# OpenDriveLab/MTGS

Hardware: AMD Instinct MI355X
Metric: rendered Mpix/s (fwd+bwd) @ 2M Gaussians 1920x1080 (higher is better)
Workload: dtype f32

## Files before the change

### include/mtgs_rast.h

```cpp
#ifndef MTGS_RAST_H
#define MTGS_RAST_H

#include <stddef.h>
#include <stdint.h>

#include "mtgs_crop.h"
#include "mtgs_refine_scene.h"
#include "mtgs_present.h"
#include "mtgs_lpips.h"
#include "mtgs_dino.h"
#include "mtgs_jpeg.h"
#include "mtgs_lidar.h"
#include "mtgs_frame.h"
#include "mtgs_stack.h"
#include "mtgs_jpegdec.h"
#include "mtgs_icp.h"

#ifdef __cplusplus
extern "C" {
#endif

#define MTGS_RAST_ABI_VERSION 29
#define MTGS_RAST_HOT_ABI_VERSION 7
#define MTGS_VIS_COLOR_ROWS 64
#define MTGS_BIN3_TIGHT 1
#define MTGS_BIN3_FILL_TO_M 2
#define MTGS_BIN3_FILL_TO_CAP 4
#define MTGS_BIN3_PREZEROED 8
#define MTGS_BIN3_STATUS 16

enum {
    MTGS_OK = 0,
    MTGS_EINVAL = 1,
    MTGS_ELAUNCH = 2,
    MTGS_EWORKSPACE = 3,
    MTGS_EUNSUPPORTED = 4
};

#define MTGS_TILE_SIZE 16
// ... 465 lines not shown
```

### mtgs_amd/_lib.py

```python
from __future__ import annotations

import ctypes as C
from pathlib import Path

import torch

from . import _abi

_PKG = Path(__file__).resolve().parent
LIB_PATH = _PKG / "libmtgs_rast.so"


def use_library(path) -> None:
    global LIB_PATH
    if _lib is not None:
        raise RuntimeError("use_library() after the library was loaded")
    LIB_PATH = Path(path)

_PROTOTYPES = {_abi.HEADER.name: _abi.prototypes()}
for _name in _abi.included_headers():
    _PROTOTYPES[_name] = _abi.header_abi(_name).prototypes
GROUPS = {header: list(group) for header, group in _PROTOTYPES.items()}
EXPORTS = GROUPS[_abi.HEADER.name]
ABI_VERSION = _abi.constant("MTGS_RAST_ABI_VERSION")
# ... 18 lines not shown
            fn.restype = restype
    v = lib.mtgs_rast_version()
    if v != ABI_VERSION:
        raise RuntimeError(f"libmtgs_rast.so ABI version {v} != expected {ABI_VERSION}; rebuild")
    if lib.mtgs_rast_hot_version() != HOT_ABI_VERSION:
        raise RuntimeError(f"libmtgs_rast.so hot-path ABI version {lib.mtgs_rast_hot_version()} != expected {HOT_ABI_VERSION}; rebuild")
    _lib = lib
    return lib


def ptr(t):
    return None if t is None else t.data_ptr()


def host_i64(values):
    return None if values is None else (C.c_int64 * len(values))(*values)


def stream_of(t: torch.Tensor):
    return torch.cuda.current_stream(t.device).cuda_stream


_timed: dict = {}


def time_calls(names=()) -> None:
    _timed.clear()
    for n in names:
        _timed[n] = []


def timed_ms() -> dict:
    return {n: [s.elapsed_time(e) for s, e in evs] for n, evs in _timed.items()}


def call(name: str, *args) -> None:
    evs = _timed.get(name) if _timed else None
    if evs is not None:
        s, e = torch.cuda.Event(enable_timing=True), torch.cuda.Event(enable_timing=True)
        s.record()
    rc = getattr(load(), name)(*args)
    if evs is not None:
        e.record()
        evs.append((s, e))
    if rc != 0:
        msg = load().mtgs_rast_last_error().decode("utf-8", "replace")
        raise RuntimeError(f"{name} failed (code {rc}): {msg}")


def size_query(name: str, *dims) -> int:
    n = C.c_size_t(0)
    call(name, *dims, C.byref(n))
    return n.value


def workspace(name: str, *dims, device, dtype, pad: int = 0) -> torch.Tensor:
    return torch.empty(size_query(name, *dims) + pad, dtype=dtype, device=device)


_scratch: dict = {}
# ... 17 lines not shown
```

### mtgs_amd/csrc/blend.hip

```cpp
#include <stdlib.h>
#include <type_traits>
#include "common.hpp"
#include "wave_reduce.hpp"
#include "raster_rec.hpp"

#ifdef MTGS_DEV
#include "dev/blend_dev.hpp"
#else
#define MTGS_COUNT_ADD(i, v) do { } while (0)
#define MTGS_COUNT_SLOTS(vmask) do { } while (0)
#define MTGS_DEV_PPL_OVERRIDE() do { } while (0)
#define MTGS_TL_DECL() do { } while (0)
#define MTGS_TL_STAGED(n) do { } while (0)
#define MTGS_TL_ACTIVE() do { } while (0)
#define MTGS_TL_END(kind) do { } while (0)
#endif

namespace {

constexpr float kAlphaMax = MTGS_ALPHA_MAX;
constexpr float kTMin = MTGS_T_MIN;
constexpr float kNoClampOpacity = 0.9989f;
constexpr float kHalfLog2e = MTGS_HALF_LOG2E;

// ... 189 lines not shown
extern "C" int mtgs_fill_zero(void *p, size_t bytes, void *stream);
inline int zero_fill_fallback(void *&also_zero, size_t also_zero_bytes, int64_t tiles, hipStream_t st) {
    if (!also_zero || also_zero_bytes == 0 || also_zero_bytes / (size_t)(tiles > 0 ? tiles : 1) <= ZERO_FILL_MAX_PER_TILE) return MTGS_OK;
    void *p = also_zero;
    also_zero = nullptr;
    return mtgs_fill_zero(p, also_zero_bytes, (void *)st);
}
inline ZeroFill make_zero_fill(void *also_zero, size_t also_zero_bytes, unsigned grid, int waves_per_block) {
    ZeroFill zf{nullptr, 0ull, 0u};
    if (also_zero && also_zero_bytes) {
        const unsigned long long n16 = also_zero_bytes / 16, waves = (unsigned long long)grid * waves_per_block;
        zf = ZeroFill{(uint4 *)also_zero, n16, (uint32_t)((n16 + waves - 1) / waves)};
    }
    return zf;
}

template <int D, int PPL, bool PK>
__global__ __launch_bounds__(256 / PPL, (PPL == 4 && D <= 4) ? MTGS_FWD_WAVES : 1) void blend_fwd_kernel(
    int C, const float *__restrict__ recs, const float *__restrict__ means2d, const float *__restrict__ conics,
    const float *__restrict__ colors, const float *__restrict__ opacities,
    const float *__restrict__ backgrounds, const float *__restrict__ depths, int DC, int ed, int W, int H,
    int tw, int th, const int32_t *__restrict__ offsets, const int32_t *__restrict__ flatten_ids, int64_t M,
    float *__restrict__ render, float *__restrict__ alphas, int32_t *__restrict__ last_ids,
    const int32_t *__restrict__ order, const ZeroFill zf) {
    constexpr int NT = 256 / PPL, ROWS = NT / 16, REC = Rec<D>::N;
    constexpr bool CULL = true;
    constexpr int CAND = NT == 64 ? 128 : 256, NR = CAND / NT;
    __shared__ __attribute__((aligned(16))) float s_rec[CAND * REC];
    __shared__ int s_wc[NT / 64];
    MTGS_TL_DECL();
    const int64_t n_tiles = (int64_t)tw * th, total_tiles = (int64_t)C * n_tiles;
    const int64_t tile = block_to_tile(order);
    const int cam = (int)(tile / n_tiles);
    const int t_in = (int)(tile - (int64_t)cam * n_tiles);
    const int ty = t_in / tw, tx = t_in - ty * tw;
    const int tid = threadIdx.x, lx = tid & 15, ly = tid >> 4;
    const int ix = tx * 16 + lx;
    const float px = (float)ix + 0.5f;
    int iy[PPL];
    float py[PPL], T[PPL], acc[PPL][D];
    int32_t last[PPL];
    unsigned long long done[PPL];
    bool inside[PPL];
#pragma unroll
    for (int p = 0; p < PPL; ++p) {
        iy[p] = ty * 16 + ly + p * ROWS;
        py[p] = (float)iy[p] + 0.5f;
        inside[p] = ix < W && iy[p] < H;
        done[p] = __ballot(!inside[p]);
        T[p] = 1.f;
        last[p] = 0;
#pragma unroll
        for (int k = 0; k < D; ++k) acc[p][k] = 0.f;
// ... 23 lines not shown
        for (int r = 0; r < NR; ++r)
            if (b0 + CAND + r * NT + tid < end) g_next[r] = flatten_ids[b0 + CAND + r * NT + tid];
        __syncthreads();
        auto entry = [&](const float4 &r0, const float4 &r1, const uint32_t va, auto off_tag, auto clamp_tag) -> bool {
            constexpr int OFF = decltype(off_tag)::value;
            constexpr bool CLAMP = decltype(clamp_tag)::value;
            ColorRow<D, REC> col;
            col.template load_at<OFF * REC * 4>(va, py[0]);
            const float dx = r0.x - px;
            const float adx = r0.z * dx, bdx = r0.w * dx;
            const float q0 = adx * dx, b2dx = bdx + bdx;
            float s2[PPL];
            unsigned long long vmask[PPL], any = 0;
#pragma unroll
            for (int p = 0; p < PPL; ++p) {
                s2[p] = eval_s2(q0, b2dx, r1.x, r0.y - py[p]);
                vmask[p] = in_range_mask(s2[p], r1.z) & ~done[p];
                any |= vmask[p];
            }
            col.wait();
            if (any == 0) return false;
            MTGS_TL_ACTIVE();
            const int32_t idx = __float_as_int(r1.w);
            unsigned long long stopped = 0;
#pragma unroll
            for (int p = 0; p < PPL; ++p) {
                if (vmask[p] != 0) {
                    const float e = __builtin_amdgcn_exp2f(-s2[p]);
                    const float alpha = CLAMP ? fminf(kAlphaMax, alpha_rounded(r1.y, e)) : alpha_rounded(r1.y, e);
                    const float w = alpha * T[p];
                    const float next_T = T[p] * (1.f - alpha);
                    const unsigned long long sm = __builtin_amdgcn_fcmpf(next_T, kTMin, 5 ) & vmask[p];
                    done[p] |= sm;
                    stopped |= sm;
                    const bool upd = __builtin_amdgcn_inverse_ballot_w64(vmask[p] & ~sm);
                    const float wu = upd ? w : 0.f;
#pragma unroll
                    for (int k = 0; k < D; ++k) acc[p][k] = fmaf(col[k], wu, acc[p][k]);
                    T[p] = upd ? next_T : T[p];
                    last[p] = upd ? idx : last[p];
                }
            }
            if (stopped) {
                unsigned long long ad = done[0];
#pragma unroll
                for (int p = 1; p < PPL; ++p) ad &= done[p];
                return ad == ~0ull;
            }
            return false;
        };
        auto run = [&](auto clamp_tag) {
            using Z = std::integral_constant<int, 0>;
            using O = std::integral_constant<int, 1>;
            const uint32_t rec0 = lds_offset(s_rec);
            auto rec_at = [&](uint32_t va, int q) {
                const f32x4 v = *reinterpret_cast<const __attribute__((address_space(3))) f32x4 *>((uintptr_t)(va + 16 * q));
                return make_float4(v.x, v.y, v.z, v.w);
            };
            uint32_t va;
            asm volatile("v_mov_b32 %0, %1" : "=v"(va) : "s"(rec0));
            float4 ra0 = rec_at(va, 0), ra1 = rec_at(va, 1), rb0 = ra0, rb1 = ra1;
            bool fin = false;
            for (int t = 0; t < bsz && !fin; t += 2) {
                asm volatile("v_mov_b32 %0, %1" : "=v"(va) : "s"(rec0 + (uint32_t)t * (REC * 4)));
                if (t + 1 < bsz) { rb0 = rec_at(va, REC / 4); rb1 = rec_at(va, REC / 4 + 1); }
                fin = entry(ra0, ra1, va, Z{}, clamp_tag);
// ... 1 lines not shown
                    if (t + 2 < bsz) { ra0 = rec_at(va, 2 * (REC / 4)); ra1 = rec_at(va, 2 * (REC / 4) + 1); }
                    fin = entry(rb0, rb1, va, O{}, clamp_tag);
                }
            }
        };
        if (may_clamp) run(std::true_type{}); else run(std::false_type{});
    }
#pragma unroll
    for (int p = 0; p < PPL; ++p) {
        if (inside[p]) {
            const int64_t pid = ((int64_t)cam * H + iy[p]) * W + ix;
            const float alpha_out = 1.f - T[p];
            alphas[pid] = alpha_out;
            last_ids[pid] = last[p];
#pragma unroll
            for (int k = 0; k < D; ++k) {
                float v = (backgrounds && k < DC) ? acc[p][k] + T[p] * backgrounds[cam * DC + k] : acc[p][k];
                if (ed && k == D - 1) v = v / fmaxf(alpha_out, 1e-10f);
                render[pid * D + k] = v;
            }
        }
    }
    zero_fill_slice<NT>(zf);
    MTGS_TL_END(0);
}

template <int PPL>
__global__ __launch_bounds__(256 / PPL) void blend_touch_kernel(int C, const float *__restrict__ recs, int W, int H, int tw, int th,
                                                                const int32_t *__restrict__ offsets,
                                                                const int32_t *__restrict__ rank_ids,
                                                                const int32_t *__restrict__ order, uint8_t *__restrict__ touched) {
    constexpr int NT = 256 / PPL, ROWS = NT / 16, REC = Rec<0>::N;
    constexpr int CAND = NT == 64 ? 128 : 256, NR = CAND / NT;
    static_assert(REC == 8, "geometry half of the record");
    __shared__ __attribute__((aligned(16))) float s_rec[CAND * REC];
    __shared__ int32_t s_id[CAND];
    __shared__ int s_wc[NT / 64];
    const int64_t n_tiles = (int64_t)tw * th;
    const int64_t tile = block_to_tile(order);
    const int cam = (int)(tile / n_tiles);
    const int t_in = (int)(tile - (int64_t)cam * n_tiles);
    const int ty = t_in / tw, tx = t_in - ty * tw;
    const int tid = threadIdx.x, lx = tid & 15, ly = tid >> 4;
    const int ix = tx * 16 + lx;
    const float px = (float)ix + 0.5f;
    float py[PPL], T[PPL];
// ... 319 lines not shown
            }
        };
        if (may_clamp) run(std::true_type{}); else run(std::false_type{});
        if (BATCH_FLUSH) {
            __syncthreads();
            for (int e = tid; e < bsz * 16; e += NT) {
                const int t = e >> 4;
                float v = 0.f;
#pragma unroll
                for (int w = 0; w < NW; ++w) v += s_grad[(w * CAND + t) * 16 + j];
                if (a_base && v != 0.f) unsafeAtomicAdd(row_address(a_base, (uint32_t)s_id[t], a_stride_bytes), v);
            }
        }
    }
    zero_slice();
}

template <int D, int PPL, bool PK = false>
int launch_fwd(int C, const float *recs, const float *means2d, const float *conics, const float *colors,
               const float *opacities, const float *backgrounds, const float *depths, int DC, int ed, int W,
               int H, int tw, int th,
               const int32_t *offsets, const int32_t *flatten_ids, int64_t M, float *render,
               float *alphas, int32_t *last_ids, const int32_t *order, hipStream_t st, void *also_zero = nullptr,
               size_t also_zero_bytes = 0) {
    const int64_t total = (int64_t)C * tw * th;
    const unsigned grid = (unsigned)total;
    blend_fwd_kernel<D, PPL, PK><<<grid, 256 / PPL, 0, st>>>(C, recs, means2d, conics, colors, opacities,
                                                         backgrounds, depths, DC, ed, W, H, tw, th, offsets,
                                                         flatten_ids, M, render, alphas, last_ids, order,
                                                         make_zero_fill(also_zero, also_zero_bytes, grid, 256 / PPL / 64));
    return 0;
}

template <int D, int PPL, bool PK = false>
int launch_bwd(int C, const float *recs, const float *means2d, const float *conics, const float *colors,
               const float *opacities, const float *backgrounds, const float *depths, int DC, int ed, int W,
               int H, int tw, int th, const int32_t *offsets, const int32_t *flatten_ids, int64_t M,
               const float *alphas, const int32_t *last_ids, const float *render, const float *v_render,
               const float *v_alphas, float *v_means2d, float *v_means2d_abs, float *v_conics, float *v_colors,
               float *v_depths, float *v_opacities, const GradRowBytes gs, const int32_t *row_index, const int32_t *order,
               hipStream_t st, void *also_zero = nullptr, size_t also_zero_bytes = 0) {
    const int64_t total = (int64_t)C * tw * th;
    const unsigned grid = (unsigned)total;
    const ZeroFill zf = make_zero_fill(also_zero, also_zero_bytes, grid, 256 / PPL / 64);
    blend_bwd_kernel<D, PPL, PK><<<grid, 256 / PPL, 0, st>>>(
        C, recs, means2d, conics, colors, opacities, backgrounds, depths, DC, ed, W, H, tw, th, offsets, flatten_ids, M,
        alphas, last_ids, render, v_render, v_alphas, v_means2d, v_means2d_abs, v_conics, v_colors, v_depths,
        v_opacities, gs, row_index, order, zf);
    return 0;
}

constexpr int SCHED_THREADS = 1024, SCHED_BUCKETS = 1024;
__global__ __launch_bounds__(SCHED_THREADS) void tile_schedule_kernel(int total_tiles, const int32_t *__restrict__ offsets,
                                                                     int64_t M, int32_t *__restrict__ order) {
    __shared__ int hist[SCHED_BUCKETS];
    __shared__ int wsum[SCHED_THREADS / 64];
    const int tid = threadIdx.x;
    hist[tid] = 0;
    __syncthreads();
    auto bucket_of = [&](int t) {
        const int64_t end = (t == total_tiles - 1) ? M : (int64_t)offsets[t + 1];
        const int len = (int)(end - offsets[t]);
        return SCHED_BUCKETS - 1 - min(len >> 2, SCHED_BUCKETS - 1);
    };
    for (int t = tid; t < total_tiles; t += SCHED_THREADS) atomicAdd(&hist[bucket_of(t)], 1);
    __syncthreads();
    const int v = hist[tid];
    int inc = v;
#pragma unroll
    for (int o = 1; o < 64; o <<= 1) {
        const int up = __shfl_up(inc, o, 64);
        if ((tid & 63) >= o) inc += up;
    }
    if ((tid & 63) == 63) wsum[tid >> 6] = inc;
    __syncthreads();
    int base = 0;
    for (int w = 0; w < (tid >> 6); ++w) base += wsum[w];
    __syncthreads();
    hist[tid] = base + inc - v;
    __syncthreads();
    for (int t = tid; t < total_tiles; t += SCHED_THREADS) order[atomicAdd(&hist[bucket_of(t)], 1)] = t;
}

bool supported_channels(int D) { return (D >= 1 && D <= 8) || D == 16 || D == 32; }

}

static int pick_ppl(int64_t total_tiles, int DT, bool backward) {
    if (DT > 8) return 1;
    MTGS_DEV_PPL_OVERRIDE();
    if (backward) {
        if (total_tiles >= 6000) return 4;
        return (DT <= 4 && total_tiles < 1536) ? 1 : 2;
    }
    return total_tiles >= 16000 ? 4 : (total_tiles >= 3000 ? 2 : 1);
}

#define MTGS_DISPATCH_ONE(FN, DD, ...)                                         \
    if (ppl == 4) FN<DD, 4>(__VA_ARGS__);                                      \
    else if (ppl == 2) FN<DD, 2>(__VA_ARGS__);                                 \
    else FN<DD, 1>(__VA_ARGS__);

#define MTGS_DISPATCH_D(FN, ...)                                      \
    switch (DT) {                                                     \
        case 1: MTGS_DISPATCH_ONE(FN, 1, __VA_ARGS__) break;          \
        case 2: MTGS_DISPATCH_ONE(FN, 2, __VA_ARGS__) break;          \
        case 3: MTGS_DISPATCH_ONE(FN, 3, __VA_ARGS__) break;          \
        case 4: MTGS_DISPATCH_ONE(FN, 4, __VA_ARGS__) break;          \
        case 5: MTGS_DISPATCH_ONE(FN, 5, __VA_ARGS__) break;          \
        case 6: MTGS_DISPATCH_ONE(FN, 6, __VA_ARGS__) break;          \
        case 7: MTGS_DISPATCH_ONE(FN, 7, __VA_ARGS__) break;          \
        case 8: MTGS_DISPATCH_ONE(FN, 8, __VA_ARGS__) break;          \
        case 16: FN<16, 1>(__VA_ARGS__); break;                       \
        default: FN<32, 1>(__VA_ARGS__); break;                       \
    }

extern "C" int mtgs_blend_fwd(int C, int64_t N, int D, const float *means2d, const float *conics,
                              const float *colors, const float *opacities, const float *backgrounds,
                              const float *depths, int ed_normalize, int width, int height, int tile_size,
                              int tile_w, int tile_h, const int32_t *offsets, const int32_t *flatten_ids,
                              int64_t M, float *render, float *alphas, int32_t *last_ids,
// ... 57 lines not shown
                    v_means2d, v_means2d_abs, v_conics, v_colors, v_depths, v_opacities, gs, grad_row_index, tile_order,
                    st);
    MTGS_CHECK_LAUNCH("mtgs_blend_bwd");
    return MTGS_OK;
}

#define MTGS_DISPATCH_PK_ONE(FN, DD, ...)                                      \
    if (ppl == 4) FN<DD, 4, true>(__VA_ARGS__);                                \
    else if (ppl == 2) FN<DD, 2, true>(__VA_ARGS__);                           \
    else FN<DD, 1, true>(__VA_ARGS__);

#define MTGS_DISPATCH_PK(FN, ...)                                     \
    switch (DT) {                                                     \
        case 1: MTGS_DISPATCH_PK_ONE(FN, 1, __VA_ARGS__) break;       \
        case 2: MTGS_DISPATCH_PK_ONE(FN, 2, __VA_ARGS__) break;       \
        case 3: MTGS_DISPATCH_PK_ONE(FN, 3, __VA_ARGS__) break;       \
        case 4: MTGS_DISPATCH_PK_ONE(FN, 4, __VA_ARGS__) break;       \
        case 5: MTGS_DISPATCH_PK_ONE(FN, 5, __VA_ARGS__) break;       \
        case 6: MTGS_DISPATCH_PK_ONE(FN, 6, __VA_ARGS__) break;       \
        case 7: MTGS_DISPATCH_PK_ONE(FN, 7, __VA_ARGS__) break;       \
        default: MTGS_DISPATCH_PK_ONE(FN, 8, __VA_ARGS__) break;      \
    }

extern "C" int mtgs_blend_fwd_packed(int C, int D, int with_depth, const float *recs, const float *backgrounds,
                                     int ed_normalize, int width, int height, int tile_w, int tile_h,
                                     const int32_t *offsets, const int32_t *rank_ids, float *render, float *alphas,
                                     int32_t *last_ids, const int32_t *tile_order, void *also_zero, size_t also_zero_bytes,
                                     void *stream) {
    MTGS_REQUIRE(C >= 0 && D >= 0 && width > 0 && height > 0, MTGS_EINVAL, "mtgs_blend_fwd_packed: bad sizes");
    MTGS_REQUIRE(!also_zero || ((reinterpret_cast<uintptr_t>(also_zero) | also_zero_bytes) & 15) == 0, MTGS_EINVAL,
                 "mtgs_blend_fwd_packed: also_zero must be a 16-byte aligned region of whole 16-byte words");
    MTGS_REQUIRE(tile_w == (width + 15) / 16 && tile_h == (height + 15) / 16, MTGS_EINVAL,
                 "mtgs_blend_fwd_packed: tile grid %dx%d does not match image %dx%d", tile_w, tile_h, width, height);
    const int DT = D + (with_depth ? 1 : 0);
    MTGS_REQUIRE(DT >= 1 && DT <= REC_MAX_CHANNELS, MTGS_EUNSUPPORTED, "mtgs_blend_fwd_packed: %d blended channels (1..%d)", DT,
                 REC_MAX_CHANNELS);
    MTGS_REQUIRE(!ed_normalize || with_depth, MTGS_EINVAL, "mtgs_blend_fwd_packed: ed_normalize needs the depth channel");
    if (C == 0) return also_zero ? mtgs_zero_async(also_zero, also_zero_bytes, (hipStream_t)stream) : MTGS_OK;
    MTGS_REQUIRE(recs && offsets && rank_ids && render && alphas && last_ids, MTGS_EINVAL, "mtgs_blend_fwd_packed: null pointer");
    hipStream_t st = (hipStream_t)stream;
    if (int rc = zero_fill_fallback(also_zero, also_zero_bytes, (int64_t)C * tile_w * tile_h, st)) return rc;
    const int ppl = pick_ppl((int64_t)C * tile_w * tile_h, DT, false);
    MTGS_DISPATCH_PK(launch_fwd, C, recs, nullptr, nullptr, nullptr, nullptr, backgrounds, nullptr, D, ed_normalize, width, height,
                     tile_w, tile_h, offsets, rank_ids, (int64_t)-1, render, alphas, last_ids, tile_order, st, also_zero, also_zero_bytes);
    MTGS_CHECK_LAUNCH("mtgs_blend_fwd_packed");
    return MTGS_OK;
}

extern "C" int mtgs_blend_touch_packed(int C, const float *recs, int width, int height, int tile_w, int tile_h, const int32_t *offsets,
                                       const int32_t *rank_ids, const int32_t *tile_order, uint8_t *touched, int64_t cap_vis,
                                       void *stream) {
    MTGS_REQUIRE(C >= 0 && width > 0 && height > 0 && cap_vis >= 0, MTGS_EINVAL, "mtgs_blend_touch_packed: bad sizes");
    MTGS_REQUIRE(tile_w == (width + 15) / 16 && tile_h == (height + 15) / 16, MTGS_EINVAL,
                 "mtgs_blend_touch_packed: tile grid %dx%d does not match image %dx%d", tile_w, tile_h, width, height);
    if (C == 0 || cap_vis == 0) return MTGS_OK;
    MTGS_REQUIRE(recs && offsets && rank_ids && touched, MTGS_EINVAL, "mtgs_blend_touch_packed: null pointer");
    hipStream_t st = (hipStream_t)stream;
    hipError_t e = hipMemsetAsync(touched, 0, (size_t)cap_vis, st);
    MTGS_REQUIRE(e == hipSuccess, MTGS_ELAUNCH, "mtgs_blend_touch_packed: memset failed");
    const int64_t total_tiles = (int64_t)C * tile_w * tile_h;
    const int ppl = pick_ppl(total_tiles, 4, false);
    const unsigned grid = (unsigned)total_tiles;
    if (ppl == 4) blend_touch_kernel<4><<<grid, 64, 0, st>>>(C, recs, width, height, tile_w, tile_h, offsets, rank_ids, tile_order, touched);
    else if (ppl == 2) blend_touch_kernel<2><<<grid, 128, 0, st>>>(C, recs, width, height, tile_w, tile_h, offsets, rank_ids, tile_order, touched);
    else blend_touch_kernel<1><<<grid, 256, 0, st>>>(C, recs, width, height, tile_w, tile_h, offsets, rank_ids, tile_order, touched);
    MTGS_CHECK_LAUNCH("mtgs_blend_touch_packed");
    return MTGS_OK;
}

// ... 22 lines not shown
    const uint32_t sb = (uint32_t)(row_stride * 4);
    const GradRowBytes gs{sb, sb, sb, sb, sb, sb};
    if (int rc = zero_fill_fallback(also_zero, also_zero_bytes, (int64_t)C * tile_w * tile_h, st)) return rc;
    const int ppl = pick_ppl((int64_t)C * tile_w * tile_h, DT, true);
    MTGS_DISPATCH_PK(launch_bwd, C, recs, nullptr, nullptr, nullptr, nullptr, backgrounds, nullptr, D, ed_normalize, width, height,
                     tile_w, tile_h, offsets, rank_ids, (int64_t)-1, alphas, last_ids, render, v_render, v_alphas, grad_rows,
                     absgrad ? grad_rows + 2 : nullptr, grad_rows + 4, grad_rows + 8, grad_rows + 8 + D, grad_rows + 7, gs, nullptr,
                     tile_order, st, also_zero, also_zero_bytes);
    MTGS_CHECK_LAUNCH("mtgs_blend_bwd_packed");
    return MTGS_OK;
}

extern "C" int mtgs_tile_schedule(int C, int tile_w, int tile_h, const int32_t *offsets, int64_t M,
                                  int32_t *tile_order, void *stream) {
    MTGS_REQUIRE(C >= 0 && tile_w > 0 && tile_h > 0 && M >= 0, MTGS_EINVAL, "mtgs_tile_schedule: bad sizes");
    const int64_t total = (int64_t)C * tile_w * tile_h;
    if (total == 0) return MTGS_OK;
    MTGS_REQUIRE(total < ((int64_t)1 << 31), MTGS_EINVAL, "mtgs_tile_schedule: too many tiles");
    MTGS_REQUIRE(offsets && tile_order, MTGS_EINVAL, "mtgs_tile_schedule: null pointer");
    tile_schedule_kernel<<<1, SCHED_THREADS, 0, (hipStream_t)stream>>>((int)total, offsets, M, tile_order);
    MTGS_CHECK_LAUNCH("mtgs_tile_schedule");
    return MTGS_OK;
}
```

### mtgs_amd/wrapper.py

```python
from __future__ import annotations

import ctypes as C
import os
import contextlib
import threading
import time
import weakref
from typing import NamedTuple, Optional, Tuple

import torch
from torch import Tensor

from . import _lib
from ._abi import constant
from ._lib import call, host_i64, ptr, require_gpu, stream_of

SUPPORTED_CHANNELS = (1, 2, 3, 4, 5, 6, 7, 8, 16, 32)
MAX_CHANNELS = 32


def _f32c(t: Optional[Tensor]) -> Optional[Tensor]:
    if t is None:
        return None
    if t.dtype != torch.float32:
        raise TypeError(f"expected float32 tensor, got {t.dtype}")
    return t.contiguous()


def _strided_rows(t: Optional[Tensor], width: int):
    if t is None:
        return None, width
    if t.dtype != torch.float32:
        raise TypeError(f"expected float32 tensor, got {t.dtype}")
    Cn, N = t.shape[:2]
    rs = t.stride(1)
    ok = rs >= width and (t.dim() == 2 or t.stride(2) == 1 or width == 1) and (Cn == 1 or t.stride(0) == N * rs)
    if N <= 1 or not ok:
# ... 603 lines not shown
        G = torch.zeros((Cn, N, RS), dtype=torch.float32, device=m2d.device)
        v_means2d, v_abs_buf, v_conics, v_opacities = G[..., 0:2], G[..., 2:4], G[..., 4:7], G[..., 7]
        v_colors = G[..., 8:8 + DC] if DC else None
        v_depths = G[..., 8 + DC] if dep is not None else None
        v_abs = v_abs_buf if ctx.absgrad else None
        call("mtgs_blend_bwd", Cn, N, DC, ptr(m2d), ptr(con), ptr(col), ptr(opa), ptr(bg), ptr(dep), int(ed),
             width, height, tile_size, tw, th, ptr(isect_offsets), ptr(flatten_ids), flatten_ids.numel(),
             ptr(alphas), ptr(last_ids), ptr(render), ptr(v_render), ptr(v_alphas), ptr(v_means2d), ptr(v_abs),
             ptr(v_conics), ptr(v_colors), ptr(v_depths), ptr(v_opacities), host_i64([RS] * 6), None, ptr(order),
             stream_of(m2d))
        if ctx.absgrad:
            ctx.means2d_ref.absgrad = v_abs
        v_bg = None
        if bg is not None and ctx.needs_input_grad[4]:
            v_bg = (v_render[..., :DC] * (1.0 - alphas)).sum(dim=(1, 2))
        return (v_means2d, v_conics, v_colors, v_opacities, v_bg, v_depths, None, None, None, None, None, None, None)


TILE_SIZE = 16
RECORD_CHANNELS = 8
_BIN3_TIGHT, _BIN3_FILL_TO_M, _BIN3_FILL_TO_CAP, _BIN3_PREZEROED, _BIN3_STATUS = (
    constant("MTGS_BIN3_" + k) for k in ("TIGHT", "FILL_TO_M", "FILL_TO_CAP", "PREZEROED", "STATUS"))
_VIS_COLOR_ROWS = constant("MTGS_VIS_COLOR_ROWS")
speculative_sizing = True
_force_caps = None
_debug_rows = None


class _SizePlan(threading.local):

    def __init__(self):
        self.seen = {}

    def caps(self, key, total):
        rec = self.seen.get(key)
        if rec is None:
            return None
        n_vis, M = rec
        cap_vis = min(total, max(4096, n_vis + n_vis // 2))
        cap_M = max(1 << 16, M + M // 2)
        return cap_vis, -(-cap_M // (1 << 16)) * (1 << 16)

    def update(self, key, n_vis, M):
        old = self.seen.get(key)
        if old is not None:
            n_vis, M = max(n_vis, old[0] - old[0] // 16), max(M, old[1] - old[1] // 16)
# ... 116 lines not shown


class _TileLists(NamedTuple):
    rank_ids: Tensor
    flatten_ids: Tensor
    isect_ids: Tensor


def _packed_path(ins, dims, outs, need, dp, cs):
    means, quats, scales, opacities, col, viewmats, Ks, bg = ins
    Cn, N, width, height, tw, th, DC, with_depth, ed, eps2d, near_plane, far_plane, radius_clip = dims
    radii, means2d, depths, conics, comps, opac_eff, tiles_per_gauss, render, alphas, last_ids = outs
    dev, st = means.device, stream_of(means)
    n2c = None if cs is None else cs.camera_normals
    zero_rows = zero_coeffs = None
    total = Cn * N
    key = (Cn, N, width, height)
    front_ws = _lib.workspace("mtgs_front_workspace_bytes", total, device=dev, dtype=torch.uint8)
    graph_caps = _graph.caps
    totals = torch.empty(4 if graph_caps is not None else 1, dtype=torch.int64, device=dev)
    vis_rank = torch.empty(total, dtype=torch.int32, device=dev)
    offsets_buf = torch.empty(Cn * th * tw + 1, dtype=torch.int32, device=dev)
    order = torch.empty(Cn * th * tw, dtype=torch.int32, device=dev)
    if graph_caps is not None and _graph.owner != threading.get_ident():
        raise RuntimeError("rasterization(): mtgs_amd.graph_mode is active on another thread (fixed capacities, no host "
                           "read-back); serialise the two callers or leave graph_mode first")

    touch_first = cs is not None and bool(cs.touch_first)
    tight = lists_are_tight()
    list_flags = (_BIN3_TIGHT if tight else 0) | (_BIN3_FILL_TO_CAP | _BIN3_STATUS if graph_caps is not None
                                                  else (_BIN3_FILL_TO_M if tight else 0))

    def colours(b, flags):
        cap_vis = b.cap_vis
        if cs.wild:
            cs.colour_rows(b.vis_ids, totals, cap_vis, b.recs, flags, st)
        else:
            coef = cs.prepare(vis_rank, cap_vis, b.vis_ids, totals, row_flags=flags)
            call("mtgs_vis_color_fwd_dirs", cs.n_nodes, ptr(cs.table), cs.degree, ptr(cs.cam), ptr(means), ptr(b.vis_ids),
                 ptr(totals), cap_vis, ptr(b.recs), ptr(b.vis_mask), ptr(coef), 0 if coef is None else coef.stride(0),
                 ptr(flags), ptr(cs.dirs), st)
        if n2c is not None:
            call("mtgs_normals_fwd_rows", cap_vis, ptr(b.vis_ids), ptr(totals), ptr(quats), ptr(scales), ptr(means),
                 ptr(n2c), ptr(b.recs), 3, ptr(flags), st)

    def bin_ws(cap_vis, cap_M):
# ... 27 lines not shown
                         torch.empty(cap_alloc, dtype=torch.int64, device=dev))
        ws, ws_ptr, ws_bytes, _ = prezeroed if prezeroed is not None else bin_ws(b.cap_vis, cap_M)
        call("mtgs_bin3_build", Cn, N, TILE_SIZE, tw, th, ptr(totals), b.cap_vis, cap_M, ptr(b.recs),
             ptr(b.vis_ids), ptr(b.vis_keys), ptr(out.rank_ids),
             ptr(out.flatten_ids), ptr(out.isect_ids), ptr(offsets_buf), ptr(order),
             list_flags | (_BIN3_PREZEROED if prezeroed is not None else 0), ws_ptr, ws_bytes, st)
        if touch_first:
            flags = torch.empty(max(b.cap_vis, 1), dtype=torch.uint8, device=dev)
            call("mtgs_blend_touch_packed", Cn, ptr(b.recs), width, height, tw, th, ptr(offsets_buf), ptr(out.rank_ids),
                 ptr(order), ptr(flags), b.cap_vis, st)
            colours(b, flags)
        z_ptr, z_bytes = None, 0
        if _prefill.enabled and _prefill.in_forward and any(need) and dp is None and zero_rows is None:
            RS = _row_stride(DC + with_depth)
            n_rows = max(b.cap_vis, 1) * RS
            n_coef = N * 48 if (cs is not None and cs.autograd and cs.width == 48 and (cs.n_nodes == 1 or cs.dirs is not None)
                                and (graph_caps is None or cs.dirs is not None) and _needs_coeffs(need, cs)) else 0
            z_ptr, z_bytes, own = _prefill.take(dev, n_rows + n_coef, only=getattr(_sh_scope, "reqs", ()))
            zero_rows = own[:n_rows].view(max(b.cap_vis, 1), RS)
            if n_coef:
                zero_coeffs = own[n_rows:].view(N, 16, 3)
        elif dp is not None and dp.zero_region is not None and any(need):
            z_ptr, z_bytes = dp.zero_region
        call("mtgs_blend_fwd_packed", Cn, DC, with_depth, ptr(b.recs), ptr(bg), int(ed), width, height, tw, th,
             ptr(offsets_buf), ptr(out.rank_ids), ptr(render), ptr(alphas), ptr(last_ids), ptr(order), z_ptr, z_bytes, st)
        return out

    caps = _force_caps or (_size_plan.caps(key, total) if speculative_sizing else None)
    if caps is not None and not _bin3_ok(Cn, tw, th, caps[1]):
        caps = None
    if graph_caps is not None:
        if dp is not None or not _bin3_ok(Cn, tw, th, graph_caps[1]):
            raise NotImplementedError("graph_mode: unsupported configuration (data-parallel exchange / capacity >= 2^30)")
        pz = bin_ws(min(graph_caps[0], total), graph_caps[1])
        b = front(min(graph_caps[0], total), prezero=pz)
        out = rest(b, graph_caps[1], prezeroed=pz)
        n_vis, M = b.cap_vis, graph_caps[1]
    elif caps is not None:
        pz = bin_ws(min(caps[0], total), caps[1])
        b = front(min(caps[0], total), prezero=pz)
        out = rest(b, caps[1], prezeroed=pz)
        n_vis, M = _wait_mailbox(b.mailbox, b.tag, totals, total)
        if n_vis > b.cap_vis or M > caps[1]:
            if not _bin3_ok(Cn, tw, th, M):
                raise NotImplementedError(f"rasterization: {M} tile intersections in one call (limit 2^30)")
            if n_vis > b.cap_vis:
                b = front(n_vis, repeat=True)
            out = rest(b, M)
    else:
        b = front(total)
        n_vis, M = _wait_mailbox(b.mailbox, b.tag, totals, total)
        if not _bin3_ok(Cn, tw, th, M):
            raise NotImplementedError(f"rasterization: {M} tile intersections in one call (limit 2^30)")
        b.cap_vis = max(n_vis, 0)
        out = rest(b, M)
    if graph_caps is None:
        _size_plan.update(key, n_vis, M)
    isect_ids = out.isect_ids[:M]
    offsets = offsets_buf[:Cn * th * tw].view(Cn, th, tw)
    offsets._mtgs_tile_order = order
    if tight or graph_caps is not None:
        offsets._mtgs_n_listed = offsets_buf[Cn * th * tw]
    isect_ids._mtgs_offsets = offsets
    return (isect_ids, out.flatten_ids[:M], offsets, offsets_buf, order, b.vis_ids[:n_vis], vis_rank, totals, b.recs, out.rank_ids[:M],
            b.vis_mask, b.cap_vis, zero_rows, zero_coeffs)


class _BackwardPlan(NamedTuple):
    want_m2d: bool
    want_abs: bool
    want_col: bool
    c0: int
    rows_only: bool
    geo_rows: bool
    zeroed: bool
    floats: int
    views: dict


def _backward_plan(*, packed, Cn, N, n_vis, DC, absgrad, has_dp, info_grads, m2d_alive, m2d_retains, need_colors, open_channels,
                   geometry_rows, want_grad_rows, prefill_enabled, zeroed_outputs) -> _BackwardPlan:
    rows_only, c0 = bool(want_grad_rows), open_channels
    want_m2d = bool(m2d_alive and m2d_retains)
    want_abs = bool(absgrad and m2d_alive and not rows_only)
    want_col = bool(DC > c0 and need_colors)
    geo_rows = bool(geometry_rows and not info_grads and n_vis > 0)
    zeroed = bool(prefill_enabled and zeroed_outputs and packed and Cn == 1 and not has_dp and n_vis > 0 and N > 0
# ... 396 lines not shown
```

Measured before the change: 2627.

## Schedule backward tiles by measured forward work instead of list length

The forward blend kernel now records, per tile, how many candidate entries and pixel strips did useful work before saturation. A new single-block kernel then buckets tiles by a weighted work estimate, heaviest first, to produce the tile order used by the backward pass. The old order was based on intersection-list length. The aim is better load balance in the backward pass, since it only walks up to the last contributing Gaussian. The cost is extra counters and a small reduction in the forward kernel, plus one more launch.

```diff
diff --git a/include/mtgs_rast.h b/include/mtgs_rast.h
--- a/include/mtgs_rast.h
+++ b/include/mtgs_rast.h
@@ -15,6 +15,7 @@
 #include "mtgs_stack.h"
 #include "mtgs_jpegdec.h"
 #include "mtgs_icp.h"
+#include "mtgs_sched.h"
 
 #ifdef __cplusplus
 extern "C" {
diff --git a/include/mtgs_sched.h b/include/mtgs_sched.h
--- /dev/null
+++ b/include/mtgs_sched.h
@@ -0,0 +1,24 @@
+#ifndef MTGS_SCHED_H
+#define MTGS_SCHED_H
+
+#include <stddef.h>
+#include <stdint.h>
+
+#ifdef __cplusplus
+extern "C" {
+#endif
+
+#define MTGS_SCHED_W_ENTRY 3
+#define MTGS_SCHED_W_STRIP 2
+int mtgs_blend_fwd_packed_work(int C, int D, int with_depth, const float *recs, const float *backgrounds,
+                               int ed_normalize, int width, int height, int tile_w, int tile_h,
+                               const int32_t *offsets, const int32_t *rank_ids, float *render, float *alphas,
+                               int32_t *last_ids, const int32_t *tile_order, void *also_zero, size_t also_zero_bytes,
+                               int32_t *tile_work, void *stream);
+int mtgs_tile_schedule_work(int64_t total_tiles, const int32_t *tile_work, int w_entry, int w_strip, int32_t *tile_order,
+                            void *stream);
+
+#ifdef __cplusplus
+}
+#endif
+#endif
diff --git a/mtgs_amd/_lib.py b/mtgs_amd/_lib.py
--- a/mtgs_amd/_lib.py
+++ b/mtgs_amd/_lib.py
@@ -64,6 +64,7 @@
 
 
 _timed: dict = {}
+_TIMED_AS = {"mtgs_blend_fwd_packed_work": "mtgs_blend_fwd_packed"}
 
 
 def time_calls(names=()) -> None:
@@ -77,7 +78,7 @@
 
 
 def call(name: str, *args) -> None:
-    evs = _timed.get(name) if _timed else None
+    evs = _timed.get(_TIMED_AS.get(name, name)) if _timed else None
     if evs is not None:
         s, e = torch.cuda.Event(enable_timing=True), torch.cuda.Event(enable_timing=True)
         s.record()
diff --git a/mtgs_amd/csrc/blend.hip b/mtgs_amd/csrc/blend.hip
--- a/mtgs_amd/csrc/blend.hip
+++ b/mtgs_amd/csrc/blend.hip
@@ -235,13 +235,15 @@
     const float *__restrict__ backgrounds, const float *__restrict__ depths, int DC, int ed, int W, int H,
     int tw, int th, const int32_t *__restrict__ offsets, const int32_t *__restrict__ flatten_ids, int64_t M,
     float *__restrict__ render, float *__restrict__ alphas, int32_t *__restrict__ last_ids,
-    const int32_t *__restrict__ order, const ZeroFill zf) {
+    const int32_t *__restrict__ order, const ZeroFill zf, int32_t *__restrict__ tile_work) {
     constexpr int NT = 256 / PPL, ROWS = NT / 16, REC = Rec<D>::N;
     constexpr bool CULL = true;
     constexpr int CAND = NT == 64 ? 128 : 256, NR = CAND / NT;
     __shared__ __attribute__((aligned(16))) float s_rec[CAND * REC];
     __shared__ int s_wc[NT / 64];
+    __shared__ int s_work[2 * (NT / 64)];
     MTGS_TL_DECL();
+    int work_entries = 0, work_strips = 0;
     const int64_t n_tiles = (int64_t)tw * th, total_tiles = (int64_t)C * n_tiles;
     const int64_t tile = block_to_tile(order);
     const int cam = (int)(tile / n_tiles);
@@ -311,7 +313,8 @@
             if (any == 0) return false;
             MTGS_TL_ACTIVE();
             const int32_t idx = __float_as_int(r1.w);
-            unsigned long long stopped = 0;
+            unsigned long long stopped = 0, updated = 0;
+            if (PPL > 1) work_entries += 1;
 #pragma unroll
             for (int p = 0; p < PPL; ++p) {
                 if (vmask[p] != 0) {
@@ -320,17 +323,24 @@
                     const float w = alpha * T[p];
                     const float next_T = T[p] * (1.f - alpha);
                     const unsigned long long sm = __builtin_amdgcn_fcmpf(next_T, kTMin, 5 ) & vmask[p];
-                    done[p] |= sm;
-                    stopped |= sm;
-                    const bool upd = __builtin_amdgcn_inverse_ballot_w64(vmask[p] & ~sm);
+                    const unsigned long long um = vmask[p] & ~sm;
+                    if (sm != 0) {
+                        done[p] |= sm;
+                        stopped |= sm;
+                        work_strips -= um == 0;
+                    }
+                    const bool upd = __builtin_amdgcn_inverse_ballot_w64(um);
                     const float wu = upd ? w : 0.f;
 #pragma unroll
                     for (int k = 0; k < D; ++k) acc[p][k] = fmaf(col[k], wu, acc[p][k]);
                     T[p] = upd ? next_T : T[p];
                     last[p] = upd ? idx : last[p];
+                    work_strips += 1;
+                    if (PPL > 1) updated |= um;
                 }
             }
             if (stopped) {
+                if (PPL > 1) work_entries -= updated == 0;
                 unsigned long long ad = done[0];
 #pragma unroll
                 for (int p = 1; p < PPL; ++p) ad &= done[p];
@@ -378,6 +388,21 @@
         }
     }
     zero_fill_slice<NT>(zf);
+    if (PPL == 1) work_entries = work_strips;
+    if (tile_work) {
+        if (NT == 64) {
+            if (tid == 0) { tile_work[2 * tile] = work_entries; tile_work[2 * tile + 1] = work_strips; }
+        } else {
+            if ((tid & 63) == 0) { s_work[2 * (tid >> 6)] = work_entries; s_work[2 * (tid >> 6) + 1] = work_strips; }
+            __syncthreads();
+            if (tid == 0) {
+                int e = 0, s = 0;
+#pragma unroll
+                for (int w = 0; w < NT / 64; ++w) { e += s_work[2 * w]; s += s_work[2 * w + 1]; }
+                tile_work[2 * tile] = e; tile_work[2 * tile + 1] = s;
+            }
+        }
+    }
     MTGS_TL_END(0);
 }
 
@@ -743,13 +768,13 @@
                int H, int tw, int th,
                const int32_t *offsets, const int32_t *flatten_ids, int64_t M, float *render,
                float *alphas, int32_t *last_ids, const int32_t *order, hipStream_t st, void *also_zero = nullptr,
-               size_t also_zero_bytes = 0) {
+               size_t also_zero_bytes = 0, int32_t *tile_work = nullptr) {
     const int64_t total = (int64_t)C * tw * th;
     const unsigned grid = (unsigned)total;
     blend_fwd_kernel<D, PPL, PK><<<grid, 256 / PPL, 0, st>>>(C, recs, means2d, conics, colors, opacities,
                                                          backgrounds, depths, DC, ed, W, H, tw, th, offsets,
                                                          flatten_ids, M, render, alphas, last_ids, order,
-                                                         make_zero_fill(also_zero, also_zero_bytes, grid, 256 / PPL / 64));
+                                                         make_zero_fill(also_zero, also_zero_bytes, grid, 256 / PPL / 64), tile_work);
     return 0;
 }
 
@@ -771,7 +796,7 @@
     return 0;
 }
 
-constexpr int SCHED_THREADS = 1024, SCHED_BUCKETS = 1024;
+constexpr int SCHED_THREADS = 1024, SCHED_BUCKETS = 1024, SCHED_CACHE = 8;
 __global__ __launch_bounds__(SCHED_THREADS) void tile_schedule_kernel(int total_tiles, const int32_t *__restrict__ offsets,
                                                                      int64_t M, int32_t *__restrict__ order) {
     __shared__ int hist[SCHED_BUCKETS];
@@ -803,6 +828,71 @@
     for (int t = tid; t < total_tiles; t += SCHED_THREADS) order[atomicAdd(&hist[bucket_of(t)], 1)] = t;
 }
 
+__global__ __launch_bounds__(SCHED_THREADS) void tile_schedule_work_kernel(int total_tiles, const int32_t *__restrict__ work,
+                                                                          int w_entry, int w_strip, int32_t *__restrict__ order) {
+    __shared__ int hist[SCHED_BUCKETS];
+    __shared__ int wsum[SCHED_THREADS / 64];
+    __shared__ unsigned long long wmax[SCHED_THREADS / 64];
+    const int tid = threadIdx.x;
+    hist[tid] = 0;
+    auto key_of = [&](int t) {
+        const long long e = max(work[2 * (int64_t)t], 0), s = max(work[2 * (int64_t)t + 1], 0);
+        return (unsigned long long)(e * w_entry + s * w_strip);
+    };
+    unsigned long long kc[SCHED_CACHE];
+    unsigned long long kmax = 0;
+#pragma unroll
+    for (int i = 0; i < SCHED_CACHE; ++i) {
+        const int t = i * SCHED_THREADS + tid;
+        kc[i] = t < total_tiles ? key_of(t) : 0ull;
+        kmax = max(kmax, kc[i]);
+    }
+    for (int t = SCHED_CACHE * SCHED_THREADS + tid; t < total_tiles; t += SCHED_THREADS) kmax = max(kmax, key_of(t));
+#pragma unroll
+    for (int o = 32; o > 0; o >>= 1) kmax = max(kmax, (unsigned long long)__shfl_xor((long long)kmax, o, 64));
+    if ((tid & 63) == 0) wmax[tid >> 6] = kmax;
+    __syncthreads();
+    kmax = 0;
+#pragma unroll
+    for (int w = 0; w < SCHED_THREADS / 64; ++w) kmax = max(kmax, wmax[w]);
+    const bool narrow = kmax * (SCHED_BUCKETS - 1) < (1ull << 32);
+    auto bucket_of_key = [&](unsigned long long key) {
+        if (kmax == 0) return SCHED_BUCKETS - 1;
+        const unsigned long long k = key * (SCHED_BUCKETS - 1);
+        const int b = narrow ? (int)((uint32_t)k / (uint32_t)kmax) : (int)(k / kmax);
+        return SCHED_BUCKETS - 1 - b;
+    };
+    auto bucket_of = [&](int t) { return bucket_of_key(key_of(t)); };
+    int bc[SCHED_CACHE];
+#pragma unroll
+    for (int i = 0; i < SCHED_CACHE; ++i) {
+        bc[i] = bucket_of_key(kc[i]);
+        if (i * SCHED_THREADS + tid < total_tiles) atomicAdd(&hist[bc[i]], 1);
+    }
+    for (int t = SCHED_CACHE * SCHED_THREADS + tid; t < total_tiles; t += SCHED_THREADS) atomicAdd(&hist[bucket_of(t)], 1);
+    __syncthreads();
+    const int v = hist[tid];
+    int inc = v;
+#pragma unroll
+    for (int o = 1; o < 64; o <<= 1) {
+        const int up = __shfl_up(inc, o, 64);
+        if ((tid & 63) >= o) inc += up;
+    }
+    if ((tid & 63) == 63) wsum[tid >> 6] = inc;
+    __syncthreads();
+    int base = 0;
+    for (int w = 0; w < (tid >> 6); ++w) base += wsum[w];
+    __syncthreads();
+    hist[tid] = base + inc - v;
+    __syncthreads();
+#pragma unroll
+    for (int i = 0; i < SCHED_CACHE; ++i) {
+        const int t = i * SCHED_THREADS + tid;
+        if (t < total_tiles) order[atomicAdd(&hist[bc[i]], 1)] = t;
+    }
+    for (int t = SCHED_CACHE * SCHED_THREADS + tid; t < total_tiles; t += SCHED_THREADS) order[atomicAdd(&hist[bucket_of(t)], 1)] = t;
+}
+
 bool supported_channels(int D) { return (D >= 1 && D <= 8) || D == 16 || D == 32; }
 
 }
@@ -817,7 +907,10 @@
     return total_tiles >= 16000 ? 4 : (total_tiles >= 3000 ? 2 : 1);
 }
 
-#define MTGS_DISPATCH_ONE(FN, DD, ...)                                         \
+static_assert(MTGS_SCHED_W_ENTRY >= 0 && MTGS_SCHED_W_ENTRY <= 65535 && MTGS_SCHED_W_STRIP >= 0 && MTGS_SCHED_W_STRIP <= 65535,
+              "mtgs_tile_schedule_work's range");
+
+#define MTGS_DISPATCH_ONE(FN, DD, ...)                                       \
     if (ppl == 4) FN<DD, 4>(__VA_ARGS__);                                      \
     else if (ppl == 2) FN<DD, 2>(__VA_ARGS__);                                 \
     else FN<DD, 1>(__VA_ARGS__);
@@ -921,29 +1014,38 @@
         default: MTGS_DISPATCH_PK_ONE(FN, 8, __VA_ARGS__) break;      \
     }
 
+static int blend_fwd_packed(const char *fn, int C, int D, int with_depth, const float *recs, const float *backgrounds,
+                            int ed_normalize, int width, int height, int tile_w, int tile_h, const int32_t *offsets,
+                            const int32_t *rank_ids, float *render, float *alphas, int32_t *last_ids,
+                            const int32_t *tile_order, void *also_zero, size_t also_zero_bytes, int32_t *tile_work,
+                            void *stream) {
+    MTGS_REQUIRE(C >= 0 && D >= 0 && width > 0 && height > 0, MTGS_EINVAL, "%s: bad sizes", fn);
+    MTGS_REQUIRE(!also_zero || ((reinterpret_cast<uintptr_t>(also_zero) | also_zero_bytes) & 15) == 0, MTGS_EINVAL,
+                 "%s: also_zero must be a 16-byte aligned region of whole 16-byte words", fn);
+    MTGS_REQUIRE(tile_w == (width + 15) / 16 && tile_h == (height + 15) / 16, MTGS_EINVAL,
+                 "%s: tile grid %dx%d does not match image %dx%d", fn, tile_w, tile_h, width, height);
+    const int DT = D + (with_depth ? 1 : 0);
+    MTGS_REQUIRE(DT >= 1 && DT <= REC_MAX_CHANNELS, MTGS_EUNSUPPORTED, "%s: %d blended channels (1..%d)", fn, DT,
+                 REC_MAX_CHANNELS);
+    MTGS_REQUIRE(!ed_normalize || with_depth, MTGS_EINVAL, "%s: ed_normalize needs the depth channel", fn);
+    if (C == 0) return also_zero ? mtgs_zero_async(also_zero, also_zero_bytes, (hipStream_t)stream) : MTGS_OK;
+    MTGS_REQUIRE(recs && offsets && rank_ids && render && alphas && last_ids, MTGS_EINVAL, "%s: null pointer", fn);
+    hipStream_t st = (hipStream_t)stream;
+    if (int rc = zero_fill_fallback(also_zero, also_zero_bytes, (int64_t)C * tile_w * tile_h, st)) return rc;
+    const int ppl = pick_ppl((int64_t)C * tile_w * tile_h, DT, false);
+    MTGS_DISPATCH_PK(launch_fwd, C, recs, nullptr, nullptr, nullptr, nullptr, backgrounds, nullptr, D, ed_normalize, width, height,
+                     tile_w, tile_h, offsets, rank_ids, (int64_t)-1, render, alphas, last_ids, tile_order, st, also_zero, also_zero_bytes, tile_work);
+    MTGS_CHECK_LAUNCH(fn);
+    return MTGS_OK;
+}
+
 extern "C" int mtgs_blend_fwd_packed(int C, int D, int with_depth, const float *recs, const float *backgrounds,
                                      int ed_normalize, int width, int height, int tile_w, int tile_h,
                                      const int32_t *offsets, const int32_t *rank_ids, float *render, float *alphas,
                                      int32_t *last_ids, const int32_t *tile_order, void *also_zero, size_t also_zero_bytes,
                                      void *stream) {
-    MTGS_REQUIRE(C >= 0 && D >= 0 && width > 0 && height > 0, MTGS_EINVAL, "mtgs_blend_fwd_packed: bad sizes");
-    MTGS_REQUIRE(!also_zero || ((reinterpret_cast<uintptr_t>(also_zero) | also_zero_bytes) & 15) == 0, MTGS_EINVAL,
-                 "mtgs_blend_fwd_packed: also_zero must be a 16-byte aligned region of whole 16-byte words");
-    MTGS_REQUIRE(tile_w == (width + 15) / 16 && tile_h == (height + 15) / 16, MTGS_EINVAL,
-                 "mtgs_blend_fwd_packed: tile grid %dx%d does not match image %dx%d", tile_w, tile_h, width, height);
-    const int DT = D + (with_depth ? 1 : 0);
-    MTGS_REQUIRE(DT >= 1 && DT <= REC_MAX_CHANNELS, MTGS_EUNSUPPORTED, "mtgs_blend_fwd_packed: %d blended channels (1..%d)", DT,
-                 REC_MAX_CHANNELS);
-    MTGS_REQUIRE(!ed_normalize || with_depth, MTGS_EINVAL, "mtgs_blend_fwd_packed: ed_normalize needs the depth channel");
-    if (C == 0) return also_zero ? mtgs_zero_async(also_zero, also_zero_bytes, (hipStream_t)stream) : MTGS_OK;
-    MTGS_REQUIRE(recs && offsets && rank_ids && render && alphas && last_ids, MTGS_EINVAL, "mtgs_blend_fwd_packed: null pointer");
-    hipStream_t st = (hipStream_t)stream;
-    if (int rc = zero_fill_fallback(also_zero, also_zero_bytes, (int64_t)C * tile_w * tile_h, st)) return rc;
-    const int ppl = pick_ppl((int64_t)C * tile_w * tile_h, DT, false);
-    MTGS_DISPATCH_PK(launch_fwd, C, recs, nullptr, nullptr, nullptr, nullptr, backgrounds, nullptr, D, ed_normalize, width, height,
-                     tile_w, tile_h, offsets, rank_ids, (int64_t)-1, render, alphas, last_ids, tile_order, st, also_zero, also_zero_bytes);
-    MTGS_CHECK_LAUNCH("mtgs_blend_fwd_packed");
-    return MTGS_OK;
+    return blend_fwd_packed("mtgs_blend_fwd_packed", C, D, with_depth, recs, backgrounds, ed_normalize, width, height, tile_w, tile_h,
+                            offsets, rank_ids, render, alphas, last_ids, tile_order, also_zero, also_zero_bytes, nullptr, stream);
 }
 
 extern "C" int mtgs_blend_touch_packed(int C, const float *recs, int width, int height, int tile_w, int tile_h, const int32_t *offsets,
@@ -1012,3 +1114,28 @@
     MTGS_CHECK_LAUNCH("mtgs_tile_schedule");
     return MTGS_OK;
 }
+
+extern "C" int mtgs_blend_fwd_packed_work(int C, int D, int with_depth, const float *recs, const float *backgrounds,
+                                          int ed_normalize, int width, int height, int tile_w, int tile_h,
+                                          const int32_t *offsets, const int32_t *rank_ids, float *render, float *alphas,
+                                          int32_t *last_ids, const int32_t *tile_order, void *also_zero, size_t also_zero_bytes,
+                                          int32_t *tile_work, void *stream) {
+    MTGS_REQUIRE(tile_work, MTGS_EINVAL, "mtgs_blend_fwd_packed_work: tile_work is null");
+    return blend_fwd_packed("mtgs_blend_fwd_packed_work", C, D, with_depth, recs, backgrounds, ed_normalize, width, height, tile_w,
+                            tile_h, offsets, rank_ids, render, alphas, last_ids, tile_order, also_zero, also_zero_bytes, tile_work,
+                            stream);
+}
+
+extern "C" int mtgs_tile_schedule_work(int64_t total_tiles, const int32_t *tile_work, int w_entry, int w_strip,
+                                       int32_t *tile_order, void *stream) {
+    MTGS_REQUIRE(total_tiles >= 0 && total_tiles < ((int64_t)1 << 31), MTGS_EINVAL,
+                 "mtgs_tile_schedule_work: total_tiles=%lld (0 .. 2^31 - 1)", (long long)total_tiles);
+    MTGS_REQUIRE(w_entry >= 0 && w_entry <= 65535, MTGS_EINVAL, "mtgs_tile_schedule_work: w_entry=%d (0 .. 65535)", w_entry);
+    MTGS_REQUIRE(w_strip >= 0 && w_strip <= 65535, MTGS_EINVAL, "mtgs_tile_schedule_work: w_strip=%d (0 .. 65535)", w_strip);
+    if (total_tiles == 0) return MTGS_OK;
+    MTGS_REQUIRE(tile_work, MTGS_EINVAL, "mtgs_tile_schedule_work: tile_work is null");
+    MTGS_REQUIRE(tile_order, MTGS_EINVAL, "mtgs_tile_schedule_work: tile_order is null");
+    tile_schedule_work_kernel<<<1, SCHED_THREADS, 0, (hipStream_t)stream>>>((int)total_tiles, tile_work, w_entry, w_strip, tile_order);
+    MTGS_CHECK_LAUNCH("mtgs_tile_schedule_work");
+    return MTGS_OK;
+}
diff --git a/mtgs_amd/wrapper.py b/mtgs_amd/wrapper.py
--- a/mtgs_amd/wrapper.py
+++ b/mtgs_amd/wrapper.py
@@ -12,7 +12,7 @@
 from torch import Tensor
 
 from . import _lib
-from ._abi import constant
+from ._abi import constant, header_abi
 from ._lib import call, host_i64, ptr, require_gpu, stream_of
 
 SUPPORTED_CHANNELS = (1, 2, 3, 4, 5, 6, 7, 8, 16, 32)
@@ -662,6 +662,10 @@
 _BIN3_TIGHT, _BIN3_FILL_TO_M, _BIN3_FILL_TO_CAP, _BIN3_PREZEROED, _BIN3_STATUS = (
     constant("MTGS_BIN3_" + k) for k in ("TIGHT", "FILL_TO_M", "FILL_TO_CAP", "PREZEROED", "STATUS"))
 _VIS_COLOR_ROWS = constant("MTGS_VIS_COLOR_ROWS")
+_SCHED = header_abi("mtgs_sched.h").constants
+_bwd_order = os.environ.get("MTGS_BWD_ORDER", "work")
+if _bwd_order not in ("work", "length"):
+    raise ValueError(f"MTGS_BWD_ORDER={_bwd_order!r}: 'work' or 'length'")
 speculative_sizing = True
 _force_caps = None
 _debug_rows = None
@@ -824,6 +828,9 @@
     vis_rank = torch.empty(total, dtype=torch.int32, device=dev)
     offsets_buf = torch.empty(Cn * th * tw + 1, dtype=torch.int32, device=dev)
     order = torch.empty(Cn * th * tw, dtype=torch.int32, device=dev)
+    by_work = _bwd_order == "work"
+    tile_work = torch.empty((Cn * th * tw, 2), dtype=torch.int32, device=dev) if by_work else None
+    bwd_order = torch.empty(Cn * th * tw, dtype=torch.int32, device=dev) if by_work else order
     if graph_caps is not None and _graph.owner != threading.get_ident():
         raise RuntimeError("rasterization(): mtgs_amd.graph_mode is active on another thread (fixed capacities, no host "
                            "read-back); serialise the two callers or leave graph_mode first")
@@ -897,8 +904,15 @@
                 zero_coeffs = own[n_rows:].view(N, 16, 3)
         elif dp is not None and dp.zero_region is not None and any(need):
             z_ptr, z_bytes = dp.zero_region
-        call("mtgs_blend_fwd_packed", Cn, DC, with_depth, ptr(b.recs), ptr(bg), int(ed), width, height, tw, th,
-             ptr(offsets_buf), ptr(out.rank_ids), ptr(render), ptr(alphas), ptr(last_ids), ptr(order), z_ptr, z_bytes, st)
+        if by_work:
+            call("mtgs_blend_fwd_packed_work", Cn, DC, with_depth, ptr(b.recs), ptr(bg), int(ed), width, height, tw, th,
+                 ptr(offsets_buf), ptr(out.rank_ids), ptr(render), ptr(alphas), ptr(last_ids), ptr(order), z_ptr, z_bytes,
+                 ptr(tile_work), st)
+            call("mtgs_tile_schedule_work", Cn * th * tw, ptr(tile_work), _SCHED["MTGS_SCHED_W_ENTRY"], _SCHED["MTGS_SCHED_W_STRIP"],
+                 ptr(bwd_order), st)
+        else:
+            call("mtgs_blend_fwd_packed", Cn, DC, with_depth, ptr(b.recs), ptr(bg), int(ed), width, height, tw, th,
+                 ptr(offsets_buf), ptr(out.rank_ids), ptr(render), ptr(alphas), ptr(last_ids), ptr(order), z_ptr, z_bytes, st)
         return out
 
     caps = _force_caps or (_size_plan.caps(key, total) if speculative_sizing else None)
@@ -937,7 +951,7 @@
     if tight or graph_caps is not None:
         offsets._mtgs_n_listed = offsets_buf[Cn * th * tw]
     isect_ids._mtgs_offsets = offsets
-    return (isect_ids, out.flatten_ids[:M], offsets, offsets_buf, order, b.vis_ids[:n_vis], vis_rank, totals, b.recs, out.rank_ids[:M],
+    return (isect_ids, out.flatten_ids[:M], offsets, offsets_buf, bwd_order, b.vis_ids[:n_vis], vis_rank, totals, b.recs, out.rank_ids[:M],
             b.vis_mask, b.cap_vis, zero_rows, zero_coeffs)
 
 
```

Result: no change. 2610 (-0.7%).
